# thu-pacman/chitu

Hardware: AMD Instinct MI355X
Metric: output tok/s (bs=16) DeepSeek-R1 FP8 TP=8; HBM GB/s vs peak (higher is better)
Workload: dtype fp8_e4m3 weights+activations (W8A8, fp32 accumulate), bf16 attention

## Files before the change

chitu_amd/csrc/moe.hip:

```cpp
#include "common.h"
#include "gemm_common.h"
#ifndef CHITU_MOE_PROBE_MASK
#define CHITU_MOE_PROBE_MASK 0
#endif

namespace chitu {

struct MoeStage {
    W8Frag w;
    i32x4 x[2];
    float xs, ws;
};

__device__ __forceinline__ void moe_store_tile(bf16_t* out_row, int n0, int g, int N, const f32x4& acc, float rw) {
#pragma unroll
    for (int h = 0; h < 2; ++h) {
        const int n = n0 + h * 8 + 2 * g;
        const uint16_t a = f32_to_bf16(acc[2 * h] * rw), b = f32_to_bf16(acc[2 * h + 1] * rw);
        if (n + 1 < N && (N & 1) == 0) *reinterpret_cast<uint32_t*>(out_row + n) = (uint32_t)a | ((uint32_t)b << 16);
        else {
            if (n < N) out_row[n] = a;
            if (n + 1 < N) out_row[n + 1] = b;
        }
    }
}

__device__ __forceinline__ float moe_routed_weight(const void* topk_w, int w_dt, int slot) {
    if (w_dt == 0) return bf16_to_f32(((const bf16_t*)topk_w)[slot]);
    if (w_dt == 1) return f16_to_f32(((const uint16_t*)topk_w)[slot]);
    return ((const float*)topk_w)[slot];
}

template <int WK, int NW, int D>
__global__ __launch_bounds__(64 * WK * NW) void moe_gemm1_kernel(
    const fp8_t* __restrict__ Xq, const float* __restrict__ Xs, const fp8_t* __restrict__ W,
    const float* __restrict__ Ws, const int32_t* __restrict__ sorted_ids,
    const int32_t* __restrict__ expert_ids, const int32_t* __restrict__ num_post_pad,
    bf16_t* __restrict__ out, int numel, int topk, int N, int K) {
    static_assert(WK == 1 || NW == 1, "either split K or tile N inside a workgroup");
    __shared__ float red[WK > 1 ? WK * 256 : 1];
    const int mb = blockIdx.y;
    if (mb * 16 >= *num_post_pad) return;
    const int lane = threadIdx.x & 63, wave = __builtin_amdgcn_readfirstlane(threadIdx.x >> 6);
    const int j = lane & 15, g = lane >> 4;
    const int n0 = (NW > 1 ? blockIdx.x * NW + wave : blockIdx.x) * 16;
    if (NW > 1 && n0 >= N) return;
    const int KB = K >> 7;
    const int slot = sorted_ids[mb * 16 + j];
    const bool valid = slot < numel;
    const int e = expert_ids[mb];
    f32x4 acc = f32x4{0.f, 0.f, 0.f, 0.f};
    if (e >= 0) {
        const int kw = NW > 1 ? 0 : wave;
        const int kb0 = KB * kw / WK, kb1 = KB * (kw + 1) / WK;
        const int slot0 = __builtin_amdgcn_readfirstlane(slot);
        const int token = (valid ? slot : min(slot0, numel - 1)) / topk;
        const fp8_t* xp = Xq + (size_t)token * K + g * 16;
        const float* xsp = Xs + (size_t)token * KB;
        const fp8_t *wp0, *wp1;
        w8_lane_ptrs(W + (size_t)e * N * K, n0, N, K, j, g, wp0, wp1);
        const float* wsp = Ws + ((size_t)e * ((N + 127) >> 7) + (n0 >> 7)) * KB;
        auto load = [&](MoeStage& st, int kb) {
            const int off = kb << 7;
            st.w.w[0] = __builtin_nontemporal_load(reinterpret_cast<const i32x4*>(wp0 + off));
            st.w.w[1] = __builtin_nontemporal_load(reinterpret_cast<const i32x4*>(wp1 + off));
            st.x[0] = *reinterpret_cast<const i32x4*>(xp + off);
            st.x[1] = *reinterpret_cast<const i32x4*>(xp + off + 64);
            st.xs = xsp[kb];
            st.ws = wsp[kb];
        };
        auto compute = [&](const MoeStage& st) {
            const f32x4 blk = w8a8_block_dot(st.w, st.x[0], st.x[1]);
#pragma unroll
            for (int r = 0; r < 4; ++r) acc[r] += (blk[r] * st.xs) * st.ws;
        };
        MoeStage ring[D];
#pragma unroll
        for (int d = 0; d < D; ++d)
            if (kb0 + d < kb1) load(ring[d], kb0 + d);
        for (int kb = kb0; kb < kb1; kb += D) {
#pragma unroll
            for (int d = 0; d < D; ++d) {
                if (kb + d < kb1) {
                    compute(ring[d]);
                    if (kb + d + D < kb1) load(ring[d], kb + d + D);
                }
            }
        }
    }
    if (WK > 1) {
        *reinterpret_cast<f32x4*>(&red[(wave * 64 + lane) * 4]) = acc;
        __syncthreads();
        if (wave != 0) return;
        acc = f32x4{0.f, 0.f, 0.f, 0.f};
#pragma unroll
        for (int w = 0; w < WK; ++w) {
            const f32x4 v = *reinterpret_cast<const f32x4*>(&red[(w * 64 + lane) * 4]);
#pragma unroll
            for (int r = 0; r < 4; ++r) acc[r] += v[r];
        }
    }
    if (!valid) return;
    moe_store_tile(out + (size_t)slot * N, n0, g, N, acc, 1.0f);
}

struct MoeStage2 {
    W8Frag wg, wu;
    i32x4 x[2];
    float xs, wsg, wsu;
};

template <int WK, int D, bool Q = false>
__global__ __launch_bounds__(Q ? 512 : 64 * WK) void moe_gemm1_silu_kernel(
    const fp8_t* __restrict__ Xq, const float* __restrict__ Xs, const fp8_t* __restrict__ W,
    const float* __restrict__ Ws, const int32_t* __restrict__ sorted_ids,
    const int32_t* __restrict__ expert_ids, const int32_t* __restrict__ num_post_pad,
    bf16_t* __restrict__ out, int numel, int topk, int I, int K, fp8_t* __restrict__ hq = nullptr,
    float* __restrict__ hs = nullptr, float eps = 0.f) {
    static_assert(!Q || WK == 1, "the quantising epilogue owns whole K");
    __shared__ float red[WK > 1 ? WK * 512 : 1];
    __shared__ float qmax[Q ? 8 * 16 : 1];
    const int mb = blockIdx.y;
    if (mb * 16 >= *num_post_pad) return;
    const int lane = threadIdx.x & 63;
    const int wave_id = __builtin_amdgcn_readfirstlane(threadIdx.x >> 6);
    const int wave = Q ? 0 : wave_id;
    const int j = lane & 15, g = lane >> 4;
    const int n0 = (Q ? blockIdx.x * 8 + wave_id : blockIdx.x) * 16;
    const int N = 2 * I;
    const int KB = K >> 7;
    const int slot = sorted_ids[mb * 16 + j];
    const bool valid = slot < numel;
    const int e = expert_ids[mb];
    f32x4 ag = f32x4{0.f, 0.f, 0.f, 0.f}, au = f32x4{0.f, 0.f, 0.f, 0.f};
    if (e >= 0) {
        const int kb0 = KB * wave / WK, kb1 = KB * (wave + 1) / WK;
        const int slot0 = __builtin_amdgcn_readfirstlane(slot);
        const int token = (valid ? slot : min(slot0, numel - 1)) / topk;
        const fp8_t* xp = Xq + (size_t)token * K + g * 16;
        const float* xsp = Xs + (size_t)token * KB;
        if (CHITU_MOE_PROBE_MASK & 1) {
            xp = Xq + (size_t)(g * 16 + (token & 15)) * 16;
            xsp = Xs + (token & 15);
        }
        const fp8_t* Wb = W + (size_t)e * N * K;
        const fp8_t *gp0, *gp1, *up0, *up1;
        w8_lane_ptrs(Wb, n0, N, K, j, g, gp0, gp1);
        w8_lane_ptrs(Wb, I + n0, N, K, j, g, up0, up1);
        const float* wsb = Ws + (size_t)e * ((N + 127) >> 7) * KB;
        const float* wsgp = wsb + (size_t)(n0 >> 7) * KB;
        const float* wsup = wsb + (size_t)((I + n0) >> 7) * KB;
        auto load = [&](MoeStage2& st, int kb) {
            const int off = kb << 7;
            st.wg.w[0] = __builtin_nontemporal_load(reinterpret_cast<const i32x4*>(gp0 + off));
            st.wg.w[1] = __builtin_nontemporal_load(reinterpret_cast<const i32x4*>(gp1 + off));
            st.wu.w[0] = __builtin_nontemporal_load(reinterpret_cast<const i32x4*>(up0 + off));
            st.wu.w[1] = __builtin_nontemporal_load(reinterpret_cast<const i32x4*>(up1 + off));
            if (CHITU_MOE_PROBE_MASK & 1) {
                st.x[0] = *reinterpret_cast<const i32x4*>(xp + (size_t)kb * 2048);
                st.x[1] = *reinterpret_cast<const i32x4*>(xp + (size_t)kb * 2048 + 1024);
                st.xs = xsp[kb * 16];
            } else {
                st.x[0] = *reinterpret_cast<const i32x4*>(xp + off);
                st.x[1] = *reinterpret_cast<const i32x4*>(xp + off + 64);
                st.xs = xsp[kb];
            }
            st.wsg = wsgp[kb];
            st.wsu = wsup[kb];
        };
        auto compute = [&](const MoeStage2& st) {
            const f32x4 bg = w8a8_block_dot(st.wg, st.x[0], st.x[1]);
            const f32x4 bu = w8a8_block_dot(st.wu, st.x[0], st.x[1]);
#pragma unroll
            for (int r = 0; r < 4; ++r) {
                ag[r] += (bg[r] * st.xs) * st.wsg;
                au[r] += (bu[r] * st.xs) * st.wsu;
            }
        };
        MoeStage2 ring[D];
#pragma unroll
        for (int d = 0; d < D; ++d)
            if (kb0 + d < kb1) load(ring[d], kb0 + d);
        for (int kb = kb0; kb < kb1; kb += D) {
#pragma unroll
            for (int d = 0; d < D; ++d) {
                if (kb + d < kb1) {
                    compute(ring[d]);
                    if (kb + d + D < kb1) load(ring[d], kb + d + D);
                }
            }
        }
    }
    if (WK > 1) {
        *reinterpret_cast<f32x4*>(&red[(wave * 128 + lane) * 4]) = ag;
        *reinterpret_cast<f32x4*>(&red[(wave * 128 + 64 + lane) * 4]) = au;
        __syncthreads();
        if (wave != 0) return;
        ag = f32x4{0.f, 0.f, 0.f, 0.f};
        au = f32x4{0.f, 0.f, 0.f, 0.f};
#pragma unroll
        for (int w = 0; w < WK; ++w) {
            const f32x4 vg = *reinterpret_cast<const f32x4*>(&red[(w * 128 + lane) * 4]);
            const f32x4 vu = *reinterpret_cast<const f32x4*>(&red[(w * 128 + 64 + lane) * 4]);
#pragma unroll
            for (int r = 0; r < 4; ++r) {
                ag[r] += vg[r];
                au[r] += vu[r];
            }
        }
    }
    if (!Q && !valid) return;
    f32x4 h;
#pragma unroll
    for (int r = 0; r < 4; ++r) {
        const float gv = round_bf16(ag[r]), uv = round_bf16(au[r]);
        const float sl = round_bf16(gv / (1.0f + expf(-gv)));
        h[r] = round_bf16(sl * uv);
    }
    if (!Q) {
        moe_store_tile(out + (size_t)slot * I, n0, g, I, h, 1.0f);
        return;
    }
    float amax = __builtin_fmaxf(__builtin_fmaxf(__builtin_fabsf(h[0]), __builtin_fabsf(h[1])),
                                 __builtin_fmaxf(__builtin_fabsf(h[2]), __builtin_fabsf(h[3])));
    amax = __builtin_fmaxf(amax, __shfl_xor(amax, 16, 64));
    amax = __builtin_fmaxf(amax, __shfl_xor(amax, 32, 64));
    if (g == 0) qmax[wave_id * 16 + j] = amax;
    __syncthreads();
    amax = qmax[j];
#pragma unroll
    for (int w = 1; w < 8; ++w) amax = __builtin_fmaxf(amax, qmax[w * 16 + j]);
    const float sc = __builtin_fmaxf(amax, eps) / 448.0f;
    const float v[8] = {h[0], h[1], h[2], h[3], 0.f, 0.f, 0.f, 0.f};
    const uint32_t codes = (uint32_t)quant8_fp8<true>(v, sc)[0];
    if (!valid) return;
    fp8_t* qrow = hq + (size_t)slot * I + n0 + 2 * g;
    *reinterpret_cast<uint16_t*>(qrow) = (uint16_t)(codes & 0xffffu);
    *reinterpret_cast<uint16_t*>(qrow + 8) = (uint16_t)(codes >> 16);
    if (wave_id == 0 && g == 0) hs[(size_t)slot * (I >> 7) + blockIdx.x] = sc;
}

__global__ __launch_bounds__(256) void moe_silu_quant_kernel(const bf16_t* __restrict__ c1,
                                                             fp8_t* __restrict__ q,
                                                             float* __restrict__ s, int64_t rows,
                                                             int I, float eps, int act_rule) {
    const int lane16 = threadIdx.x & 15;
    const int gpr = I >> 7;
    const int64_t n_groups = rows * gpr;
    int64_t group = ((int64_t)blockIdx.x * blockDim.x + threadIdx.x) >> 4;
    const int64_t stride = ((int64_t)gridDim.x * blockDim.x) >> 4;
    for (; group < n_groups; group += stride) {
        const int64_t row = group / gpr;
        const int col = (int)(group % gpr) * 128 + lane16 * 8;
        const i32x4 graw = *reinterpret_cast<const i32x4*>(c1 + row * 2 * I + col);
        const i32x4 uraw = *reinterpret_cast<const i32x4*>(c1 + row * 2 * I + I + col);
        float h[8];
        float amax = 0.f;
#pragma unroll
        for (int i = 0; i < 8; ++i) {
            const uint32_t gu = (uint32_t)graw[i >> 1], uu = (uint32_t)uraw[i >> 1];
            const float gv = (i & 1) ? __uint_as_float(gu & 0xffff0000u) : __uint_as_float(gu << 16);
            const float uv = (i & 1) ? __uint_as_float(uu & 0xffff0000u) : __uint_as_float(uu << 16);
            const float sl = round_bf16(gv / (1.0f + expf(-gv)));
            h[i] = round_bf16(sl * uv);
            amax = __builtin_fmaxf(amax, __builtin_fabsf(h[i]));
        }
        amax = row16_reduce_max(amax);
        if (!act_rule) amax = __builtin_fmaxf(amax, eps);
        const float sc = amax / 448.0f;
        const i32x2 o = act_rule ? quant8_fp8<false>(h, sc) : quant8_fp8<true>(h, sc);
        *reinterpret_cast<i32x2*>(q + row * I + col) = o;
        if (lane16 == 0) s[group] = sc;
    }
}

template <int KBMAX, int NT>
__global__ __launch_bounds__(256) void moe_gemm2_kernel(
    const fp8_t* __restrict__ Hq, const float* __restrict__ Hs, const fp8_t* __restrict__ W,
    const float* __restrict__ Ws, const int32_t* __restrict__ sorted_ids,
    const int32_t* __restrict__ expert_ids, const int32_t* __restrict__ num_post_pad,
    const void* __restrict__ topk_w, int w_dt, bf16_t* __restrict__ out, int numel, int N, int I,
    int mul_weight) {
    const int mb = blockIdx.y;
    if (mb * 16 >= *num_post_pad) return;
    const int lane = threadIdx.x & 63, wave = __builtin_amdgcn_readfirstlane(threadIdx.x >> 6);
    const int j = lane & 15, g = lane >> 4;
    const int KB = I >> 7;
    const int slot = sorted_ids[mb * 16 + j];
    const bool valid = slot < numel;
    const int e = expert_ids[mb];
    const int row = valid ? slot : 0;
    const float rw = (mul_weight && valid) ? moe_routed_weight(topk_w, w_dt, slot) : 1.0f;
    i32x4 x[KBMAX][2];
    float xs[KBMAX];
    if (e >= 0) {
        const fp8_t* xp = Hq + (size_t)row * I + g * 16;
#pragma unroll
        for (int kb = 0; kb < KBMAX; ++kb) {
            if (kb < KB) {
                x[kb][0] = *reinterpret_cast<const i32x4*>(xp + (kb << 7));
                x[kb][1] = *reinterpret_cast<const i32x4*>(xp + (kb << 7) + 64);
                xs[kb] = Hs[(size_t)row * KB + kb];
            }
        }
    }
    const int tile0 = (blockIdx.x * 4 + wave) * NT;
    W8Frag wf[NT][KBMAX];
    if (e >= 0) {
#pragma unroll
        for (int t = 0; t < NT; ++t) {
            const int n0 = (tile0 + t) * 16;
            if (n0 < N) {
                const fp8_t *wp0, *wp1;
                w8_lane_ptrs(W + (size_t)e * N * I, n0, N, I, j, g, wp0, wp1);
#pragma unroll
                for (int kb = 0; kb < KBMAX; ++kb) {
                    if (kb < KB) {
                        wf[t][kb].w[0] = __builtin_nontemporal_load(reinterpret_cast<const i32x4*>(wp0 + (kb << 7)));
                        wf[t][kb].w[1] = __builtin_nontemporal_load(reinterpret_cast<const i32x4*>(wp1 + (kb << 7)));
                    }
                }
            }
        }
    }
#pragma unroll
    for (int t = 0; t < NT; ++t) {
        const int n0 = (tile0 + t) * 16;
        if (n0 >= N) break;
        f32x4 acc = f32x4{0.f, 0.f, 0.f, 0.f};
        if (e >= 0) {
            const float* wsp = Ws + ((size_t)e * ((N + 127) >> 7) + (n0 >> 7)) * KB;
#pragma unroll
            for (int kb = 0; kb < KBMAX; ++kb) {
                if (kb < KB) {
                    const f32x4 blk = w8a8_block_dot(wf[t][kb], x[kb][0], x[kb][1]);
                    const float ws = wsp[kb];
#pragma unroll
                    for (int r = 0; r < 4; ++r) acc[r] += (blk[r] * xs[kb]) * ws;
                }
            }
        }
        if (valid) moe_store_tile(out + (size_t)slot * N, n0, g, N, acc, rw);
    }
}

template <int KB, int NT, int ROUNDS>
__global__ __launch_bounds__(256) void moe_gemm2_q_kernel(
    const bf16_t* __restrict__ Hb, const fp8_t* __restrict__ W, const float* __restrict__ Ws,
    const int32_t* __restrict__ sorted_ids, const int32_t* __restrict__ expert_ids,
    const int32_t* __restrict__ num_post_pad, const void* __restrict__ topk_w, int w_dt,
    bf16_t* __restrict__ out, int numel, int N, int mul_weight, float eps) {
    constexpr int I = KB * 128;
    constexpr int HPW = (2 * KB + 3) / 4;
    __shared__ float amax_lds[2 * KB][16];
    __shared__ i32x4 xq_lds[2 * KB][64];
    const int mb = blockIdx.y;
    if (mb * 16 >= *num_post_pad) return;
    const int lane = threadIdx.x & 63, wave = __builtin_amdgcn_readfirstlane(threadIdx.x >> 6);
    const int j = lane & 15, g = lane >> 4;
    const int slot = sorted_ids[mb * 16 + j];
    const bool valid = slot < numel;
    const int e = expert_ids[mb];
    auto tile_of = [&](int r) { return ((blockIdx.x * ROUNDS + r) * 4 + wave) * NT; };
    if (e < 0) {
#pragma unroll
        for (int r = 0; r < ROUNDS; ++r)
#pragma unroll
            for (int t = 0; t < NT; ++t) {
                const int n0 = (tile_of(r) + t) * 16;
                if (n0 < N && valid) moe_store_tile(out + (size_t)slot * N, n0, g, N, f32x4{0.f, 0.f, 0.f, 0.f}, 1.0f);
            }
        return;
    }
    const int row = valid ? slot : 0;
    const bf16_t* hrow = Hb + (size_t)row * I;
    i32x4 hraw[HPW][2];
#pragma unroll
    for (int q = 0; q < HPW; ++q) {
        const int hb = min(wave + 4 * q, 2 * KB - 1);
        hraw[q][0] = *reinterpret_cast<const i32x4*>(hrow + hb * 64 + g * 16);
        hraw[q][1] = *reinterpret_cast<const i32x4*>(hrow + hb * 64 + g * 16 + 8);
    }
    const int last_tile = (N - 1) >> 4;
    const fp8_t* We = W + (size_t)e * N * I;
    W8Frag wf[ROUNDS > 1 ? 2 : 1][NT][KB];
    auto load_round = [&](W8Frag (&dst)[NT][KB], int r) {
#pragma unroll
        for (int t = 0; t < NT; ++t) {
            const int n0 = min(tile_of(r) + t, last_tile) * 16;
            const fp8_t *wp0, *wp1;
            w8_lane_ptrs(We, n0, N, I, j, g, wp0, wp1);
#pragma unroll
            for (int kb = 0; kb < KB; ++kb) {
                dst[t][kb].w[0] = __builtin_nontemporal_load(reinterpret_cast<const i32x4*>(wp0 + (kb << 7)));
                dst[t][kb].w[1] = __builtin_nontemporal_load(reinterpret_cast<const i32x4*>(wp1 + (kb << 7)));
            }
        }
    };
    load_round(wf[0], 0);
    const float rw = (mul_weight && valid) ? moe_routed_weight(topk_w, w_dt, slot) : 1.0f;
    float h[HPW][16];
#pragma unroll
    for (int q = 0; q < HPW; ++q) {
        const int hb = wave + 4 * q;
        float amax = 0.f;
#pragma unroll
        for (int i = 0; i < 16; ++i) {
            const uint32_t u = (uint32_t)hraw[q][i >> 3][(i >> 1) & 3];
            h[q][i] = (i & 1) ? __uint_as_float(u & 0xffff0000u) : __uint_as_float(u << 16);
            amax = __builtin_fmaxf(amax, __builtin_fabsf(h[q][i]));
        }
        amax = __builtin_fmaxf(amax, __shfl_xor(amax, 16, 64));
        amax = __builtin_fmaxf(amax, __shfl_xor(amax, 32, 64));
        if (g == 0 && hb < 2 * KB) amax_lds[hb][j] = amax;
    }
    __syncthreads();
#pragma unroll
    for (int q = 0; q < HPW; ++q) {
        const int hb = wave + 4 * q;
        if (hb < 2 * KB) {
            const float sc = __builtin_fmaxf(__builtin_fmaxf(amax_lds[hb & ~1][j], amax_lds[hb | 1][j]), eps) / 448.0f;
            float lo[8], hi[8];
#pragma unroll
            for (int i = 0; i < 8; ++i) {
                lo[i] = h[q][i];
                hi[i] = h[q][8 + i];
            }
            const i32x2 a = quant8_fp8<true>(lo, sc), b = quant8_fp8<true>(hi, sc);
            xq_lds[hb][lane] = i32x4{a[0], a[1], b[0], b[1]};
        }
    }
    __syncthreads();
    i32x4 x[KB][2];
    float xs[KB];
#pragma unroll
    for (int kb = 0; kb < KB; ++kb) {
        x[kb][0] = xq_lds[2 * kb][lane];
        x[kb][1] = xq_lds[2 * kb + 1][lane];
        xs[kb] = __builtin_fmaxf(__builtin_fmaxf(amax_lds[2 * kb][j], amax_lds[2 * kb + 1][j]), eps) / 448.0f;
    }
    const float* wse = Ws + (size_t)e * ((N + 127) >> 7) * KB;
#pragma unroll
    for (int r = 0; r < ROUNDS; ++r) {
        if (r + 1 < ROUNDS) load_round(wf[(r + 1) & 1], r + 1);
#pragma unroll
        for (int t = 0; t < NT; ++t) {
            const int n0 = (tile_of(r) + t) * 16;
            f32x4 acc = f32x4{0.f, 0.f, 0.f, 0.f};
            const float* wsp = wse + (size_t)(min(n0, N - 1) >> 7) * KB;
#pragma unroll
            for (int kb = 0; kb < KB; ++kb) {
                const f32x4 blk = w8a8_block_dot(wf[r & 1][t][kb], x[kb][0], x[kb][1]);
                const float ws = wsp[kb];
#pragma unroll
                for (int rr = 0; rr < 4; ++rr) acc[rr] += (blk[rr] * xs[kb]) * ws;
            }
            if (valid && n0 < N) moe_store_tile(out + (size_t)slot * N, n0, g, N, acc, rw);
        }
    }
}

template <int WK>
__global__ __launch_bounds__(64 * WK) void moe_gemm2_generic_kernel(
    const fp8_t* __restrict__ Hq, const float* __restrict__ Hs, const fp8_t* __restrict__ W,
    const float* __restrict__ Ws, const int32_t* __restrict__ sorted_ids,
    const int32_t* __restrict__ expert_ids, const int32_t* __restrict__ num_post_pad,
    const void* __restrict__ topk_w, int w_dt, bf16_t* __restrict__ out, int numel, int N, int I,
    int mul_weight) {
    __shared__ float red[WK > 1 ? WK * 256 : 1];
    const int mb = blockIdx.y;
    if (mb * 16 >= *num_post_pad) return;
    const int lane = threadIdx.x & 63, wave = __builtin_amdgcn_readfirstlane(threadIdx.x >> 6);
    const int j = lane & 15, g = lane >> 4;
    const int n0 = blockIdx.x * 16;
    const int KB = I >> 7;
    const int slot = sorted_ids[mb * 16 + j];
    const bool valid = slot < numel;
    const int e = expert_ids[mb];
    const int row = valid ? slot : 0;
    f32x4 acc = f32x4{0.f, 0.f, 0.f, 0.f};
    if (e >= 0) {
        const int kb0 = KB * wave / WK, kb1 = KB * (wave + 1) / WK;
        const fp8_t* xp = Hq + (size_t)row * I + g * 16;
        const float* xsp = Hs + (size_t)row * KB;
        const fp8_t *wp0, *wp1;
        w8_lane_ptrs(W + (size_t)e * N * I, n0, N, I, j, g, wp0, wp1);
        const float* wsp = Ws + ((size_t)e * ((N + 127) >> 7) + (n0 >> 7)) * KB;
        for (int kb = kb0; kb < kb1; ++kb) {
            const int off = kb << 7;
            W8Frag f;
            f.w[0] = __builtin_nontemporal_load(reinterpret_cast<const i32x4*>(wp0 + off));
            f.w[1] = __builtin_nontemporal_load(reinterpret_cast<const i32x4*>(wp1 + off));
            const i32x4 x0 = *reinterpret_cast<const i32x4*>(xp + off);
            const i32x4 x1 = *reinterpret_cast<const i32x4*>(xp + off + 64);
            const f32x4 blk = w8a8_block_dot(f, x0, x1);
            const float xs = xsp[kb], ws = wsp[kb];
#pragma unroll
            for (int r = 0; r < 4; ++r) acc[r] += (blk[r] * xs) * ws;
        }
    }
    if (WK > 1) {
        *reinterpret_cast<f32x4*>(&red[(wave * 64 + lane) * 4]) = acc;
        __syncthreads();
        if (wave != 0) return;
        acc = f32x4{0.f, 0.f, 0.f, 0.f};
#pragma unroll
        for (int w = 0; w < WK; ++w) {
            const f32x4 v = *reinterpret_cast<const f32x4*>(&red[(w * 64 + lane) * 4]);
#pragma unroll
            for (int r = 0; r < 4; ++r) acc[r] += v[r];
        }
    }
    if (!valid) return;
    const float rw = mul_weight ? moe_routed_weight(topk_w, w_dt, slot) : 1.0f;
    moe_store_tile(out + (size_t)slot * N, n0, g, N, acc, rw);
}

__global__ __launch_bounds__(256) void moe_sum_kernel(const bf16_t* __restrict__ c3,
                                                      bf16_t* __restrict__ out, int64_t M, int topk,
                                                      int64_t N) {
    const int64_t n8 = N >> 3;
    for (int64_t idx = (int64_t)blockIdx.x * blockDim.x + threadIdx.x; idx < M * n8;
         idx += (int64_t)gridDim.x * blockDim.x) {
        const int64_t t = idx / n8, c = (idx % n8) * 8;
        float acc[8] = {0.f, 0.f, 0.f, 0.f, 0.f, 0.f, 0.f, 0.f};
        for (int k = 0; k < topk; ++k) {
            const i32x4 raw = *reinterpret_cast<const i32x4*>(c3 + (t * topk + k) * N + c);
#pragma unroll
            for (int i = 0; i < 4; ++i) {
                const uint32_t u = (uint32_t)raw[i];
                acc[2 * i] += __uint_as_float(u << 16);
                acc[2 * i + 1] += __uint_as_float(u & 0xffff0000u);
            }
        }
        i32x4 o;
#pragma unroll
        for (int i = 0; i < 4; ++i)
            o[i] = (int)((uint32_t)f32_to_bf16(acc[2 * i]) | ((uint32_t)f32_to_bf16(acc[2 * i + 1]) << 16));
        *reinterpret_cast<i32x4*>(out + t * N + c) = o;
    }
}

}

extern "C" int chitu_hip_moe_gemm1_fp8(const void* a_fp8, const float* a_scale, const void* w1_fp8,
                                       const float* w1_scale, const int32_t* sorted_token_ids,
                                       const int32_t* expert_ids,
                                       const int32_t* num_tokens_post_pad, void* out_bf16,
                                       int64_t numel, int32_t topk, int64_t N, int64_t K,
                                       int64_t max_mblocks, void* stream) {
    using namespace chitu;
    CHITU_REQUIRE(a_fp8 && a_scale && w1_fp8 && w1_scale && sorted_token_ids && expert_ids);
    CHITU_REQUIRE(num_tokens_post_pad && out_bf16);
    CHITU_REQUIRE(numel >= 0 && topk >= 1 && N >= 1 && K >= 128 && max_mblocks >= 0);
    if (K % 128 != 0) return CHITU_ERR_UNSUPPORTED;
    if (numel == 0 || max_mblocks == 0) return CHITU_OK;
    const int n_tiles = (int)((N + 15) / 16);
    const dim3 grid((unsigned)n_tiles, (unsigned)max_mblocks);
    const int64_t wgs = (int64_t)n_tiles * (numel < max_mblocks ? numel : max_mblocks);
    const int KB = (int)(K / 128);
    int WK = wgs <= 512 ? 8 : wgs <= 1024 ? 4 : wgs <= 2048 ? 2 : 1;
// ... 188 lines not shown
```

chitu_amd/csrc/moe_bf16.hip:

```cpp
#include "common.h"
#include "gemm_common.h"

namespace chitu {

constexpr int kWBf16 = 0, kWSoftFp8 = 1;

template <int WKIND>
struct MoeBfStage {
    i32x4 w[2];
    s16x8 x[WKIND == kWSoftFp8 ? 4 : 2];
    float ws;
};

template <int WKIND>
struct MoeBfAcc {
    f32x4 e0, o0, e1, o1;
    __device__ __forceinline__ void zero() { e0 = o0 = e1 = o1 = f32x4{0.f, 0.f, 0.f, 0.f}; }
    __device__ __forceinline__ f32x4 fold() const { return f32x4{e0[0] + o0[1], e0[2] + o0[3], e1[0] + o1[1], e1[2] + o1[3]}; }
};

template <int WKIND>
__device__ __forceinline__ void moe_bf_mma(MoeBfAcc<WKIND>& a, const i32x4 (&w)[2], const s16x8* x, float ws) {
    if (WKIND == kWBf16) {
        const s16x8 w0 = __builtin_bit_cast(s16x8, w[0]), w1 = __builtin_bit_cast(s16x8, w[1]);
        a.e0 = __builtin_amdgcn_mfma_f32_16x16x32_bf16(w0, x[0], a.e0, 0, 0, 0);
        a.o0 = __builtin_amdgcn_mfma_f32_16x16x32_bf16(w0, x[1], a.o0, 0, 0, 0);
        a.e1 = __builtin_amdgcn_mfma_f32_16x16x32_bf16(w1, x[0], a.e1, 0, 0, 0);
        a.o1 = __builtin_amdgcn_mfma_f32_16x16x32_bf16(w1, x[1], a.o1, 0, 0, 0);
    } else {
        const float s2 = ws * __uint_as_float(0x7B800000u);
#pragma unroll
        for (int h = 0; h < 2; ++h) {
            const s16x8 wa = soft_decode8((uint32_t)w[h][0], (uint32_t)w[h][1], s2);
            const s16x8 wb = soft_decode8((uint32_t)w[h][2], (uint32_t)w[h][3], s2);
            f32x4& e = h == 0 ? a.e0 : a.e1;
            f32x4& o = h == 0 ? a.o0 : a.o1;
            e = __builtin_amdgcn_mfma_f32_16x16x32_bf16(wa, x[0], e, 0, 0, 0);
            e = __builtin_amdgcn_mfma_f32_16x16x32_bf16(wb, x[1], e, 0, 0, 0);
            o = __builtin_amdgcn_mfma_f32_16x16x32_bf16(wa, x[2], o, 0, 0, 0);
            o = __builtin_amdgcn_mfma_f32_16x16x32_bf16(wb, x[3], o, 0, 0, 0);
        }
    }
}

template <int WKIND, int WK, bool SILU>
__global__ __launch_bounds__(64 * WK) void moe_gemm_bf16_kernel(
    const bf16_t* __restrict__ X, const void* __restrict__ Wv, const float* __restrict__ Ws,
    const int32_t* __restrict__ sorted_ids, const int32_t* __restrict__ expert_ids,
    const int32_t* __restrict__ num_post_pad, const void* __restrict__ topk_w, int w_dt, int mul_routed,
    bf16_t* __restrict__ out, int numel, int a_div, int N_out, int K) {
    constexpr int kTiles = SILU ? 2 : 1;
    __shared__ float red[WK > 1 ? WK * kTiles * 256 : 1];
    const int mb = blockIdx.y;
    if (mb * 16 >= *num_post_pad) return;
    const int lane = threadIdx.x & 63, wave = __builtin_amdgcn_readfirstlane(threadIdx.x >> 6);
    const int j = lane & 15, g = lane >> 4;
    const int n0 = blockIdx.x * 16;
    const int Nw = SILU ? 2 * N_out : N_out;
    constexpr int kBlk = WKIND == kWSoftFp8 ? 128 : 64;
    constexpr int kEl = WKIND == kWSoftFp8 ? 1 : 2;
    const int KB = K / kBlk;
    const int slot = sorted_ids[mb * 16 + j];
    const bool valid = slot < numel;
    const int e = expert_ids[mb];
    MoeBfAcc<WKIND> acc[kTiles];
#pragma unroll
    for (int t = 0; t < kTiles; ++t) acc[t].zero();
    if (e >= 0) {
        const int kb0 = KB * wave / WK, kb1 = KB * (wave + 1) / WK;
        const int slot0 = __builtin_amdgcn_readfirstlane(slot);
        const int row = (valid ? slot : min(slot0, numel - 1)) / a_div;
        const bf16_t* xp = X + (size_t)row * K + g * (WKIND == kWSoftFp8 ? 16 : 8);
        const uint8_t* Wb = (const uint8_t*)Wv + (size_t)e * Nw * K * kEl;
        const int loff = ((j & 1) * 4 + g) * 16;
        const uint8_t* wp[kTiles][2];
        const float* wsp[kTiles];
#pragma unroll
        for (int t = 0; t < kTiles; ++t) {
            const int base = t * N_out + n0, lim = t * N_out + N_out - 1;
            wp[t][0] = Wb + (size_t)min(base + (j >> 1), lim) * K * kEl + loff;
            wp[t][1] = Wb + (size_t)min(base + 8 + (j >> 1), lim) * K * kEl + loff;
            wsp[t] = WKIND == kWSoftFp8 ? Ws + ((size_t)e * ((Nw + 127) >> 7) + (base >> 7)) * KB : nullptr;
        }
        constexpr int D = SILU ? 2 : 3;
        MoeBfStage<WKIND> ring[D][kTiles];
        auto load = [&](MoeBfStage<WKIND> (&st)[kTiles], int kb) {
            const size_t off = (size_t)kb * 128;
#pragma unroll
            for (int t = 0; t < kTiles; ++t) {
                st[t].w[0] = __builtin_nontemporal_load(reinterpret_cast<const i32x4*>(wp[t][0] + off));
                st[t].w[1] = __builtin_nontemporal_load(reinterpret_cast<const i32x4*>(wp[t][1] + off));
                st[t].ws = WKIND == kWSoftFp8 ? wsp[t][kb] : 1.0f;
            }
            const bf16_t* xk = xp + (size_t)kb * kBlk;
            if (WKIND == kWSoftFp8) {
                st[0].x[0] = *reinterpret_cast<const s16x8*>(xk);
                st[0].x[1] = *reinterpret_cast<const s16x8*>(xk + 8);
                st[0].x[2] = *reinterpret_cast<const s16x8*>(xk + 64);
                st[0].x[3] = *reinterpret_cast<const s16x8*>(xk + 72);
            } else {
                st[0].x[0] = *reinterpret_cast<const s16x8*>(xk);
                st[0].x[1] = *reinterpret_cast<const s16x8*>(xk + 32);
            }
        };
        auto compute = [&](const MoeBfStage<WKIND> (&st)[kTiles]) {
#pragma unroll
            for (int t = 0; t < kTiles; ++t) moe_bf_mma<WKIND>(acc[t], st[t].w, st[0].x, st[t].ws);
        };
#pragma unroll
        for (int d = 0; d < D; ++d)
            if (kb0 + d < kb1) load(ring[d], kb0 + d);
        for (int kb = kb0; kb < kb1; kb += D) {
#pragma unroll
            for (int d = 0; d < D; ++d) {
                if (kb + d < kb1) {
                    compute(ring[d]);
                    if (kb + d + D < kb1) load(ring[d], kb + d + D);
                }
            }
        }
    }
    f32x4 r[kTiles];
#pragma unroll
    for (int t = 0; t < kTiles; ++t) r[t] = acc[t].fold();
    if (WK > 1) {
#pragma unroll
        for (int t = 0; t < kTiles; ++t) *reinterpret_cast<f32x4*>(&red[((wave * kTiles + t) * 64 + lane) * 4]) = r[t];
        __syncthreads();
        if (wave != 0) return;
#pragma unroll
        for (int t = 0; t < kTiles; ++t) {
            r[t] = f32x4{0.f, 0.f, 0.f, 0.f};
#pragma unroll
            for (int w = 0; w < WK; ++w) {
                const f32x4 v = *reinterpret_cast<const f32x4*>(&red[((w * kTiles + t) * 64 + lane) * 4]);
#pragma unroll
                for (int i = 0; i < 4; ++i) r[t][i] += v[i];
            }
        }
    }
    if (!valid) return;
    f32x4 res = r[0];
    float rw = 1.0f;
    if (SILU) {
#pragma unroll
        for (int i = 0; i < 4; ++i) {
            const float gv = round_bf16(r[0][i]), uv = round_bf16(r[1][i]);
// ... 67 lines not shown
```

chitu_amd/csrc/moe_int8.hip:

```cpp
#include "common.h"
#include "gemm_common.h"

namespace chitu {

typedef int i32x4m __attribute__((ext_vector_type(4)));

struct I8Stage2 {
    i32x4m wg[2], wu[2], x[2];
};
struct I8Stage1 {
    i32x4m w[2], x[2];
};

__device__ __forceinline__ i32x4m i8_combine(const i32x4m& e0, const i32x4m& o0, const i32x4m& e1, const i32x4m& o1) {
    return i32x4m{e0[0] + o0[1], e0[2] + o0[3], e1[0] + o1[1], e1[2] + o1[3]};
}

__device__ __forceinline__ void i8_store_tile(bf16_t* row, int n0, int g, int N, const float (&v)[4]) {
#pragma unroll
    for (int h = 0; h < 2; ++h) {
        const int n = n0 + h * 8 + 2 * g;
        if (n + 1 < N && (N & 1) == 0) *reinterpret_cast<uint32_t*>(row + n) = f32x2_to_bf16x2(v[2 * h], v[2 * h + 1]);
        else {
            if (n < N) row[n] = f32_to_bf16(v[2 * h]);
            if (n + 1 < N) row[n + 1] = f32_to_bf16(v[2 * h + 1]);
        }
    }
}

template <int WK>
__global__ __launch_bounds__(64 * WK) void moe_i8_gemm1_silu_kernel(
    const int8_t* __restrict__ Xq, const float* __restrict__ Xs, const int8_t* __restrict__ W,
    const float* __restrict__ Ws, const int32_t* __restrict__ sorted_ids, const int32_t* __restrict__ expert_ids,
    const int32_t* __restrict__ num_post_pad, bf16_t* __restrict__ out, int numel, int topk, int I, int K) {
    __shared__ int red[WK > 1 ? WK * 512 : 1];
    const int mb = blockIdx.y;
    if (mb * 16 >= *num_post_pad) return;
    const int lane = threadIdx.x & 63, wave = __builtin_amdgcn_readfirstlane(threadIdx.x >> 6);
    const int j = lane & 15, g = lane >> 4;
    const int n0 = blockIdx.x * 16;
    const int N = 2 * I;
    const int KB = K >> 7;
    const int slot = sorted_ids[mb * 16 + j];
    const bool valid = slot < numel;
    const int e = expert_ids[mb];
    const int slot0 = __builtin_amdgcn_readfirstlane(slot);
    const int token = (valid ? slot : min(slot0, numel - 1)) / topk;
    i32x4m ge0 = {0, 0, 0, 0}, go0 = ge0, ge1 = ge0, go1 = ge0, ue0 = ge0, uo0 = ge0, ue1 = ge0, uo1 = ge0;
    if (e >= 0) {
        const int kb0 = KB * wave / WK, kb1 = KB * (wave + 1) / WK;
        const int8_t* xp = Xq + (size_t)token * K + g * 16;
        const fp8_t* Wb = reinterpret_cast<const fp8_t*>(W) + (size_t)e * N * K;
        const fp8_t *gp0, *gp1, *up0, *up1;
        w8_lane_ptrs(Wb, n0, N, K, j, g, gp0, gp1);
        w8_lane_ptrs(Wb, I + n0, N, K, j, g, up0, up1);
        auto load = [&](I8Stage2& st, int kb) {
            const int off = kb << 7;
            st.wg[0] = __builtin_nontemporal_load(reinterpret_cast<const i32x4m*>(gp0 + off));
            st.wg[1] = __builtin_nontemporal_load(reinterpret_cast<const i32x4m*>(gp1 + off));
            st.wu[0] = __builtin_nontemporal_load(reinterpret_cast<const i32x4m*>(up0 + off));
            st.wu[1] = __builtin_nontemporal_load(reinterpret_cast<const i32x4m*>(up1 + off));
            st.x[0] = *reinterpret_cast<const i32x4m*>(xp + off);
            st.x[1] = *reinterpret_cast<const i32x4m*>(xp + off + 64);
        };
        auto compute = [&](const I8Stage2& st) {
            ge0 = __builtin_amdgcn_mfma_i32_16x16x64_i8(st.wg[0], st.x[0], ge0, 0, 0, 0);
            go0 = __builtin_amdgcn_mfma_i32_16x16x64_i8(st.wg[0], st.x[1], go0, 0, 0, 0);
            ge1 = __builtin_amdgcn_mfma_i32_16x16x64_i8(st.wg[1], st.x[0], ge1, 0, 0, 0);
            go1 = __builtin_amdgcn_mfma_i32_16x16x64_i8(st.wg[1], st.x[1], go1, 0, 0, 0);
            ue0 = __builtin_amdgcn_mfma_i32_16x16x64_i8(st.wu[0], st.x[0], ue0, 0, 0, 0);
            uo0 = __builtin_amdgcn_mfma_i32_16x16x64_i8(st.wu[0], st.x[1], uo0, 0, 0, 0);
            ue1 = __builtin_amdgcn_mfma_i32_16x16x64_i8(st.wu[1], st.x[0], ue1, 0, 0, 0);
            uo1 = __builtin_amdgcn_mfma_i32_16x16x64_i8(st.wu[1], st.x[1], uo1, 0, 0, 0);
        };
        constexpr int D = 3;
        I8Stage2 ring[D];
#pragma unroll
        for (int d = 0; d < D; ++d)
            if (kb0 + d < kb1) load(ring[d], kb0 + d);
        for (int kb = kb0; kb < kb1; kb += D) {
#pragma unroll
            for (int d = 0; d < D; ++d) {
                if (kb + d < kb1) {
                    compute(ring[d]);
                    if (kb + d + D < kb1) load(ring[d], kb + d + D);
                }
            }
        }
    }
    i32x4m ag = i8_combine(ge0, go0, ge1, go1), au = i8_combine(ue0, uo0, ue1, uo1);
    if (WK > 1) {
        *reinterpret_cast<i32x4m*>(&red[(wave * 128 + lane) * 4]) = ag;
        *reinterpret_cast<i32x4m*>(&red[(wave * 128 + 64 + lane) * 4]) = au;
        __syncthreads();
        if (wave != 0) return;
        ag = au = i32x4m{0, 0, 0, 0};
#pragma unroll
        for (int w = 0; w < WK; ++w) {
            const i32x4m vg = *reinterpret_cast<const i32x4m*>(&red[(w * 128 + lane) * 4]);
            const i32x4m vu = *reinterpret_cast<const i32x4m*>(&red[(w * 128 + 64 + lane) * 4]);
#pragma unroll
            for (int r = 0; r < 4; ++r) {
                ag[r] += vg[r];
                au[r] += vu[r];
            }
        }
    }
    if (!valid) return;
    const float sx = Xs[token];
    const float* wse = Ws + (size_t)max(e, 0) * N;
    float h[4];
#pragma unroll
    for (int r = 0; r < 4; ++r) {
        const int n = w8_out_col(n0, g, r);
        const int nc = min(n, I - 1);
        const float gv = e >= 0 ? round_bf16(((float)ag[r] * sx) * wse[nc]) : 0.f;
        const float uv = e >= 0 ? round_bf16(((float)au[r] * sx) * wse[I + nc]) : 0.f;
        h[r] = round_bf16(gv / (1.0f + expf(-gv))) * uv;
    }
    i8_store_tile(out + (size_t)slot * I, n0, g, I, h);
}

template <int WK>
__global__ __launch_bounds__(64 * WK) void moe_i8_gemm2_kernel(
    const int8_t* __restrict__ Aq, const float* __restrict__ As, const int8_t* __restrict__ W,
    const float* __restrict__ Ws, const int32_t* __restrict__ sorted_ids, const int32_t* __restrict__ expert_ids,
    const int32_t* __restrict__ num_post_pad, const void* __restrict__ topk_w, int w_dt, bf16_t* __restrict__ out,
    int numel, int N, int I, int mul_weight) {
    __shared__ int red[WK > 1 ? WK * 256 : 1];
    const int mb = blockIdx.y;
    if (mb * 16 >= *num_post_pad) return;
    const int lane = threadIdx.x & 63, wave = __builtin_amdgcn_readfirstlane(threadIdx.x >> 6);
    const int j = lane & 15, g = lane >> 4;
    const int n0 = blockIdx.x * 16;
    const int KB = I >> 7;
    const int slot = sorted_ids[mb * 16 + j];
    const bool valid = slot < numel;
    const int e = expert_ids[mb];
    const int row = valid ? slot : 0;
    i32x4m e0 = {0, 0, 0, 0}, o0 = e0, e1 = e0, o1 = e0;
    if (e >= 0) {
        const int kb0 = KB * wave / WK, kb1 = KB * (wave + 1) / WK;
        const int8_t* xp = Aq + (size_t)row * I + g * 16;
        const fp8_t *wp0, *wp1;
        w8_lane_ptrs(reinterpret_cast<const fp8_t*>(W) + (size_t)e * N * I, n0, N, I, j, g, wp0, wp1);
        auto load = [&](I8Stage1& st, int kb) {
            const int off = kb << 7;
            st.w[0] = __builtin_nontemporal_load(reinterpret_cast<const i32x4m*>(wp0 + off));
            st.w[1] = __builtin_nontemporal_load(reinterpret_cast<const i32x4m*>(wp1 + off));
            st.x[0] = *reinterpret_cast<const i32x4m*>(xp + off);
            st.x[1] = *reinterpret_cast<const i32x4m*>(xp + off + 64);
        };
        auto compute = [&](const I8Stage1& st) {
            e0 = __builtin_amdgcn_mfma_i32_16x16x64_i8(st.w[0], st.x[0], e0, 0, 0, 0);
            o0 = __builtin_amdgcn_mfma_i32_16x16x64_i8(st.w[0], st.x[1], o0, 0, 0, 0);
            e1 = __builtin_amdgcn_mfma_i32_16x16x64_i8(st.w[1], st.x[0], e1, 0, 0, 0);
            o1 = __builtin_amdgcn_mfma_i32_16x16x64_i8(st.w[1], st.x[1], o1, 0, 0, 0);
        };
        constexpr int D = 4;
        I8Stage1 ring[D];
#pragma unroll
        for (int d = 0; d < D; ++d)
            if (kb0 + d < kb1) load(ring[d], kb0 + d);
        for (int kb = kb0; kb < kb1; kb += D) {
#pragma unroll
            for (int d = 0; d < D; ++d) {
                if (kb + d < kb1) {
                    compute(ring[d]);
                    if (kb + d + D < kb1) load(ring[d], kb + d + D);
                }
            }
        }
    }
    i32x4m acc = i8_combine(e0, o0, e1, o1);
    if (WK > 1) {
        *reinterpret_cast<i32x4m*>(&red[(wave * 64 + lane) * 4]) = acc;
        __syncthreads();
        if (wave != 0) return;
        acc = i32x4m{0, 0, 0, 0};
#pragma unroll
        for (int w = 0; w < WK; ++w) {
            const i32x4m v = *reinterpret_cast<const i32x4m*>(&red[(w * 64 + lane) * 4]);
#pragma unroll
            for (int r = 0; r < 4; ++r) acc[r] += v[r];
        }
    }
    if (!valid) return;
    float rw = 1.0f;
    if (mul_weight)
        rw = w_dt == 0 ? bf16_to_f32(((const bf16_t*)topk_w)[slot]) : w_dt == 1 ? f16_to_f32(((const uint16_t*)topk_w)[slot]) : ((const float*)topk_w)[slot];
    const float sa = As[row];
    const float* wse = Ws + (size_t)max(e, 0) * N;
    float y[4];
#pragma unroll
    for (int r = 0; r < 4; ++r) {
        const int n = min(w8_out_col(n0, g, r), N - 1);
        y[r] = e >= 0 ? round_bf16(((float)acc[r] * sa) * wse[n]) * rw : 0.f;
    }
    i8_store_tile(out + (size_t)slot * N, n0, g, N, y);
}

static int pick_wk(int64_t wgs, int KB) {
    int WK = wgs <= 640 ? 8 : 4;
    if (KB < 16) WK = wgs <= 640 ? 8 : wgs <= 1536 ? 4 : wgs <= 3200 ? 2 : 1;
    debug_override(kOptMoeI8WK, WK);
    while (WK > 1 && WK > KB) WK >>= 1;
    return WK;
}

}

extern "C" int chitu_hip_moe_i8_gemm1_silu(const void* a_int8, const float* a_scale, const void* w1_int8,
                                           const float* w1_scale, const int32_t* sorted_token_ids,
                                           const int32_t* expert_ids, const int32_t* num_tokens_post_pad,
                                           void* h_bf16, int64_t numel, int32_t topk, int64_t inter_size, int64_t K,
                                           int64_t max_mblocks, void* stream) {
    using namespace chitu;
    CHITU_REQUIRE(a_int8 && a_scale && w1_int8 && w1_scale && sorted_token_ids && expert_ids && num_tokens_post_pad && h_bf16);
    CHITU_REQUIRE(numel >= 0 && topk >= 1 && inter_size >= 16 && K >= 128 && max_mblocks >= 0);
    if (K % 128 != 0 || inter_size % 16 != 0) return CHITU_ERR_UNSUPPORTED;
    if (numel == 0 || max_mblocks == 0) return CHITU_OK;
// ... 39 lines not shown
```

Before: 205.7.

## Hoist MoE block-head loads and issue expert weight prefetch before token gathers

Adds a shared block-head helper that loads num_post_pad and expert_ids together into scalar registers, and fetches the 16 sorted slot ids with one vector load instead of per-lane gathers. In the fused gate/up SiLU kernel and the quantising down-projection kernel, expert weight loads are issued before the dependent token-index and activation loads, so HBM weight streaming starts without waiting on the slot-to-token chain. The down-projection kernel also gets a deeper weight prefetch ring plus an occupancy hint in launch_bounds. The costs are higher register pressure, which may lower occupancy or cause spills, and inline-asm ties that constrain the compiler's scheduling.

```diff
diff --git a/chitu_amd/csrc/moe.hip b/chitu_amd/csrc/moe.hip
--- a/chitu_amd/csrc/moe.hip
+++ b/chitu_amd/csrc/moe.hip
@@ -1,5 +1,6 @@
 #include "common.h"
 #include "gemm_common.h"
+#include "moe_head.h"
 #ifndef CHITU_MOE_PROBE_MASK
 #define CHITU_MOE_PROBE_MASK 0
 #endif
@@ -40,15 +41,15 @@
     static_assert(WK == 1 || NW == 1, "either split K or tile N inside a workgroup");
     __shared__ float red[WK > 1 ? WK * 256 : 1];
     const int mb = blockIdx.y;
-    if (mb * 16 >= *num_post_pad) return;
+    int e;
+    if (!moe_block_head(expert_ids, num_post_pad, mb, e)) return;
     const int lane = threadIdx.x & 63, wave = __builtin_amdgcn_readfirstlane(threadIdx.x >> 6);
     const int j = lane & 15, g = lane >> 4;
     const int n0 = (NW > 1 ? blockIdx.x * NW + wave : blockIdx.x) * 16;
     if (NW > 1 && n0 >= N) return;
     const int KB = K >> 7;
-    const int slot = sorted_ids[mb * 16 + j];
+    const int slot = moe_block_slot(sorted_ids, mb, j);
     const bool valid = slot < numel;
-    const int e = expert_ids[mb];
     f32x4 acc = f32x4{0.f, 0.f, 0.f, 0.f};
     if (e >= 0) {
         const int kw = NW > 1 ? 0 : wave;
@@ -121,7 +122,9 @@
     __shared__ float red[WK > 1 ? WK * 512 : 1];
     __shared__ float qmax[Q ? 8 * 16 : 1];
     const int mb = blockIdx.y;
-    if (mb * 16 >= *num_post_pad) return;
+    int e;
+    if (!moe_block_head(expert_ids, num_post_pad, mb, e, Xq, Xs, W, Ws, sorted_ids, numel, topk, I, K)) return;
+    const i32x16u ids = moe_block_slots(sorted_ids, mb);
     const int lane = threadIdx.x & 63;
     const int wave_id = __builtin_amdgcn_readfirstlane(threadIdx.x >> 6);
     const int wave = Q ? 0 : wave_id;
@@ -129,45 +132,54 @@
     const int n0 = (Q ? blockIdx.x * 8 + wave_id : blockIdx.x) * 16;
     const int N = 2 * I;
     const int KB = K >> 7;
-    const int slot = sorted_ids[mb * 16 + j];
+    f32x4 ag = f32x4{0.f, 0.f, 0.f, 0.f}, au = f32x4{0.f, 0.f, 0.f, 0.f};
+    const int kb0 = KB * wave / WK, kb1 = KB * (wave + 1) / WK;
+    const fp8_t *gp0, *gp1, *up0, *up1, *xp;
+    const float *wsgp, *wsup, *xsp;
+    auto load_w = [&](MoeStage2& st, int kb) {
+        const int off = kb << 7;
+        st.wg.w[0] = __builtin_nontemporal_load(reinterpret_cast<const i32x4*>(gp0 + off));
+        st.wg.w[1] = __builtin_nontemporal_load(reinterpret_cast<const i32x4*>(gp1 + off));
+        st.wu.w[0] = __builtin_nontemporal_load(reinterpret_cast<const i32x4*>(up0 + off));
+        st.wu.w[1] = __builtin_nontemporal_load(reinterpret_cast<const i32x4*>(up1 + off));
+        st.wsg = wsgp[kb];
+        st.wsu = wsup[kb];
+    };
+    auto load_x = [&](MoeStage2& st, int kb) {
+        const int off = kb << 7;
+        if (CHITU_MOE_PROBE_MASK & 1) {
+            st.x[0] = *reinterpret_cast<const i32x4*>(xp + (size_t)kb * 2048);
+            st.x[1] = *reinterpret_cast<const i32x4*>(xp + (size_t)kb * 2048 + 1024);
+            st.xs = xsp[kb * 16];
+        } else {
+            st.x[0] = *reinterpret_cast<const i32x4*>(xp + off);
+            st.x[1] = *reinterpret_cast<const i32x4*>(xp + off + 64);
+            st.xs = xsp[kb];
+        }
+    };
+    MoeStage2 ring[D];
+    if (e >= 0) {
+        const fp8_t* Wb = W + (size_t)e * N * K;
+        w8_lane_ptrs(Wb, n0, N, K, j, g, gp0, gp1);
+        w8_lane_ptrs(Wb, I + n0, N, K, j, g, up0, up1);
+        const float* wsb = Ws + (size_t)e * ((N + 127) >> 7) * KB;
+        wsgp = wsb + (size_t)(n0 >> 7) * KB;
+        wsup = wsb + (size_t)((I + n0) >> 7) * KB;
+#pragma unroll
+        for (int d = 0; d < D; ++d)
+            if (kb0 + d < kb1) load_w(ring[d], kb0 + d);
+    }
+    const int slot = moe_slot_of_lane(ids, j);
     const bool valid = slot < numel;
-    const int e = expert_ids[mb];
-    f32x4 ag = f32x4{0.f, 0.f, 0.f, 0.f}, au = f32x4{0.f, 0.f, 0.f, 0.f};
     if (e >= 0) {
-        const int kb0 = KB * wave / WK, kb1 = KB * (wave + 1) / WK;
         const int slot0 = __builtin_amdgcn_readfirstlane(slot);
         const int token = (valid ? slot : min(slot0, numel - 1)) / topk;
-        const fp8_t* xp = Xq + (size_t)token * K + g * 16;
-        const float* xsp = Xs + (size_t)token * KB;
+        xp = Xq + (size_t)token * K + g * 16;
+        xsp = Xs + (size_t)token * KB;
         if (CHITU_MOE_PROBE_MASK & 1) {
             xp = Xq + (size_t)(g * 16 + (token & 15)) * 16;
             xsp = Xs + (token & 15);
         }
-        const fp8_t* Wb = W + (size_t)e * N * K;
-        const fp8_t *gp0, *gp1, *up0, *up1;
-        w8_lane_ptrs(Wb, n0, N, K, j, g, gp0, gp1);
-        w8_lane_ptrs(Wb, I + n0, N, K, j, g, up0, up1);
-        const float* wsb = Ws + (size_t)e * ((N + 127) >> 7) * KB;
-        const float* wsgp = wsb + (size_t)(n0 >> 7) * KB;
-        const float* wsup = wsb + (size_t)((I + n0) >> 7) * KB;
-        auto load = [&](MoeStage2& st, int kb) {
-            const int off = kb << 7;
-            st.wg.w[0] = __builtin_nontemporal_load(reinterpret_cast<const i32x4*>(gp0 + off));
-            st.wg.w[1] = __builtin_nontemporal_load(reinterpret_cast<const i32x4*>(gp1 + off));
-            st.wu.w[0] = __builtin_nontemporal_load(reinterpret_cast<const i32x4*>(up0 + off));
-            st.wu.w[1] = __builtin_nontemporal_load(reinterpret_cast<const i32x4*>(up1 + off));
-            if (CHITU_MOE_PROBE_MASK & 1) {
-                st.x[0] = *reinterpret_cast<const i32x4*>(xp + (size_t)kb * 2048);
-                st.x[1] = *reinterpret_cast<const i32x4*>(xp + (size_t)kb * 2048 + 1024);
-                st.xs = xsp[kb * 16];
-            } else {
-                st.x[0] = *reinterpret_cast<const i32x4*>(xp + off);
-                st.x[1] = *reinterpret_cast<const i32x4*>(xp + off + 64);
-                st.xs = xsp[kb];
-            }
-            st.wsg = wsgp[kb];
-            st.wsu = wsup[kb];
-        };
         auto compute = [&](const MoeStage2& st) {
             const f32x4 bg = w8a8_block_dot(st.wg, st.x[0], st.x[1]);
             const f32x4 bu = w8a8_block_dot(st.wu, st.x[0], st.x[1]);
@@ -177,16 +189,18 @@
                 au[r] += (bu[r] * st.xs) * st.wsu;
             }
         };
-        MoeStage2 ring[D];
 #pragma unroll
         for (int d = 0; d < D; ++d)
-            if (kb0 + d < kb1) load(ring[d], kb0 + d);
+            if (kb0 + d < kb1) load_x(ring[d], kb0 + d);
         for (int kb = kb0; kb < kb1; kb += D) {
 #pragma unroll
             for (int d = 0; d < D; ++d) {
                 if (kb + d < kb1) {
                     compute(ring[d]);
-                    if (kb + d + D < kb1) load(ring[d], kb + d + D);
+                    if (kb + d + D < kb1) {
+                        load_w(ring[d], kb + d + D);
+                        load_x(ring[d], kb + d + D);
+                    }
                 }
             }
         }
@@ -282,13 +296,13 @@
     const void* __restrict__ topk_w, int w_dt, bf16_t* __restrict__ out, int numel, int N, int I,
     int mul_weight) {
     const int mb = blockIdx.y;
-    if (mb * 16 >= *num_post_pad) return;
+    int e;
+    if (!moe_block_head(expert_ids, num_post_pad, mb, e)) return;
     const int lane = threadIdx.x & 63, wave = __builtin_amdgcn_readfirstlane(threadIdx.x >> 6);
     const int j = lane & 15, g = lane >> 4;
     const int KB = I >> 7;
-    const int slot = sorted_ids[mb * 16 + j];
+    const int slot = moe_block_slot(sorted_ids, mb, j);
     const bool valid = slot < numel;
-    const int e = expert_ids[mb];
     const int row = valid ? slot : 0;
     const float rw = (mul_weight && valid) ? moe_routed_weight(topk_w, w_dt, slot) : 1.0f;
     i32x4 x[KBMAX][2];
@@ -345,7 +359,7 @@
 }
 
 template <int KB, int NT, int ROUNDS>
-__global__ __launch_bounds__(256) void moe_gemm2_q_kernel(
+__global__ __launch_bounds__(256, NT <= 2 ? 3 : 1) void moe_gemm2_q_kernel(
     const bf16_t* __restrict__ Hb, const fp8_t* __restrict__ W, const float* __restrict__ Ws,
     const int32_t* __restrict__ sorted_ids, const int32_t* __restrict__ expert_ids,
     const int32_t* __restrict__ num_post_pad, const void* __restrict__ topk_w, int w_dt,
@@ -355,24 +369,51 @@
     __shared__ float amax_lds[2 * KB][16];
     __shared__ i32x4 xq_lds[2 * KB][64];
     const int mb = blockIdx.y;
-    if (mb * 16 >= *num_post_pad) return;
+    int e;
+    if (!moe_block_head(expert_ids, num_post_pad, mb, e, Hb, W, Ws, sorted_ids, topk_w, w_dt, out, numel, N, mul_weight)) return;
+    const i32x16u ids = moe_block_slots(sorted_ids, mb);
     const int lane = threadIdx.x & 63, wave = __builtin_amdgcn_readfirstlane(threadIdx.x >> 6);
     const int j = lane & 15, g = lane >> 4;
-    const int slot = sorted_ids[mb * 16 + j];
-    const bool valid = slot < numel;
-    const int e = expert_ids[mb];
     auto tile_of = [&](int r) { return ((blockIdx.x * ROUNDS + r) * 4 + wave) * NT; };
     if (e < 0) {
+        const int slot = moe_slot_of_lane(ids, j);
 #pragma unroll
         for (int r = 0; r < ROUNDS; ++r)
 #pragma unroll
             for (int t = 0; t < NT; ++t) {
                 const int n0 = (tile_of(r) + t) * 16;
-                if (n0 < N && valid) moe_store_tile(out + (size_t)slot * N, n0, g, N, f32x4{0.f, 0.f, 0.f, 0.f}, 1.0f);
+                if (n0 < N && slot < numel) moe_store_tile(out + (size_t)slot * N, n0, g, N, f32x4{0.f, 0.f, 0.f, 0.f}, 1.0f);
             }
         return;
     }
+    const int last_tile = (N - 1) >> 4;
+    const fp8_t* We = W + (size_t)e * N * I;
+    constexpr int PF = NT <= 2 ? (ROUNDS > 2 ? 2 : ROUNDS - 1) : (ROUNDS > 1 ? 1 : 0);
+    constexpr int WFD = PF + 1;
+    W8Frag wf[WFD][NT][KB];
+    auto load_round = [&](W8Frag (&dst)[NT][KB], int r) {
+#pragma unroll
+        for (int t = 0; t < NT; ++t) {
+            const int n0 = min(tile_of(r) + t, last_tile) * 16;
+            const fp8_t *wp0, *wp1;
+            w8_lane_ptrs(We, n0, N, I, j, g, wp0, wp1);
+#pragma unroll
+            for (int kb = 0; kb < KB; ++kb) {
+                dst[t][kb].w[0] = __builtin_nontemporal_load(reinterpret_cast<const i32x4*>(wp0 + (kb << 7)));
+                dst[t][kb].w[1] = __builtin_nontemporal_load(reinterpret_cast<const i32x4*>(wp1 + (kb << 7)));
+            }
+        }
+    };
+    load_round(wf[0], 0);
+    if (PF >= 2) load_round(wf[1], 1);
+    const int slot = moe_slot_of_lane(ids, j);
+    const bool valid = slot < numel;
     const int row = valid ? slot : 0;
+    uint32_t rw_bits;
+    if (mul_weight) {
+        if (w_dt == 2) rw_bits = ((const uint32_t*)topk_w)[row];
+        else rw_bits = ((const uint16_t*)topk_w)[row];
+    }
     const bf16_t* hrow = Hb + (size_t)row * I;
     i32x4 hraw[HPW][2];
 #pragma unroll
@@ -381,24 +422,6 @@
         hraw[q][0] = *reinterpret_cast<const i32x4*>(hrow + hb * 64 + g * 16);
         hraw[q][1] = *reinterpret_cast<const i32x4*>(hrow + hb * 64 + g * 16 + 8);
     }
-    const int last_tile = (N - 1) >> 4;
-    const fp8_t* We = W + (size_t)e * N * I;
-    W8Frag wf[ROUNDS > 1 ? 2 : 1][NT][KB];
-    auto load_round = [&](W8Frag (&dst)[NT][KB], int r) {
-#pragma unroll
-        for (int t = 0; t < NT; ++t) {
-            const int n0 = min(tile_of(r) + t, last_tile) * 16;
-            const fp8_t *wp0, *wp1;
-            w8_lane_ptrs(We, n0, N, I, j, g, wp0, wp1);
-#pragma unroll
-            for (int kb = 0; kb < KB; ++kb) {
-                dst[t][kb].w[0] = __builtin_nontemporal_load(reinterpret_cast<const i32x4*>(wp0 + (kb << 7)));
-                dst[t][kb].w[1] = __builtin_nontemporal_load(reinterpret_cast<const i32x4*>(wp1 + (kb << 7)));
-            }
-        }
-    };
-    load_round(wf[0], 0);
-    const float rw = (mul_weight && valid) ? moe_routed_weight(topk_w, w_dt, slot) : 1.0f;
     float h[HPW][16];
 #pragma unroll
     for (int q = 0; q < HPW; ++q) {
@@ -440,9 +463,11 @@
         xs[kb] = __builtin_fmaxf(__builtin_fmaxf(amax_lds[2 * kb][j], amax_lds[2 * kb + 1][j]), eps) / 448.0f;
     }
     const float* wse = Ws + (size_t)e * ((N + 127) >> 7) * KB;
+    float rw = 1.0f;
+    if (mul_weight && valid) rw = w_dt == 0 ? __uint_as_float(rw_bits << 16) : w_dt == 1 ? f16_to_f32((uint16_t)rw_bits) : __uint_as_float(rw_bits);
 #pragma unroll
     for (int r = 0; r < ROUNDS; ++r) {
-        if (r + 1 < ROUNDS) load_round(wf[(r + 1) & 1], r + 1);
+        if (PF >= 1 && r + PF < ROUNDS) load_round(wf[(r + PF) % WFD], r + PF);
 #pragma unroll
         for (int t = 0; t < NT; ++t) {
             const int n0 = (tile_of(r) + t) * 16;
@@ -450,7 +475,7 @@
             const float* wsp = wse + (size_t)(min(n0, N - 1) >> 7) * KB;
 #pragma unroll
             for (int kb = 0; kb < KB; ++kb) {
-                const f32x4 blk = w8a8_block_dot(wf[r & 1][t][kb], x[kb][0], x[kb][1]);
+                const f32x4 blk = w8a8_block_dot(wf[r % WFD][t][kb], x[kb][0], x[kb][1]);
                 const float ws = wsp[kb];
 #pragma unroll
                 for (int rr = 0; rr < 4; ++rr) acc[rr] += (blk[rr] * xs[kb]) * ws;
@@ -469,14 +494,14 @@
     int mul_weight) {
     __shared__ float red[WK > 1 ? WK * 256 : 1];
     const int mb = blockIdx.y;
-    if (mb * 16 >= *num_post_pad) return;
+    int e;
+    if (!moe_block_head(expert_ids, num_post_pad, mb, e)) return;
     const int lane = threadIdx.x & 63, wave = __builtin_amdgcn_readfirstlane(threadIdx.x >> 6);
     const int j = lane & 15, g = lane >> 4;
     const int n0 = blockIdx.x * 16;
     const int KB = I >> 7;
-    const int slot = sorted_ids[mb * 16 + j];
+    const int slot = moe_block_slot(sorted_ids, mb, j);
     const bool valid = slot < numel;
-    const int e = expert_ids[mb];
     const int row = valid ? slot : 0;
     f32x4 acc = f32x4{0.f, 0.f, 0.f, 0.f};
     if (e >= 0) {
diff --git a/chitu_amd/csrc/moe_bf16.hip b/chitu_amd/csrc/moe_bf16.hip
--- a/chitu_amd/csrc/moe_bf16.hip
+++ b/chitu_amd/csrc/moe_bf16.hip
@@ -1,5 +1,6 @@
 #include "common.h"
 #include "gemm_common.h"
+#include "moe_head.h"
 
 namespace chitu {
 
@@ -52,7 +53,8 @@
     constexpr int kTiles = SILU ? 2 : 1;
     __shared__ float red[WK > 1 ? WK * kTiles * 256 : 1];
     const int mb = blockIdx.y;
-    if (mb * 16 >= *num_post_pad) return;
+    int e;
+    if (!moe_block_head(expert_ids, num_post_pad, mb, e)) return;
     const int lane = threadIdx.x & 63, wave = __builtin_amdgcn_readfirstlane(threadIdx.x >> 6);
     const int j = lane & 15, g = lane >> 4;
     const int n0 = blockIdx.x * 16;
@@ -60,9 +62,8 @@
     constexpr int kBlk = WKIND == kWSoftFp8 ? 128 : 64;
     constexpr int kEl = WKIND == kWSoftFp8 ? 1 : 2;
     const int KB = K / kBlk;
-    const int slot = sorted_ids[mb * 16 + j];
+    const int slot = moe_block_slot(sorted_ids, mb, j);
     const bool valid = slot < numel;
-    const int e = expert_ids[mb];
     MoeBfAcc<WKIND> acc[kTiles];
 #pragma unroll
     for (int t = 0; t < kTiles; ++t) acc[t].zero();
diff --git a/chitu_amd/csrc/moe_head.h b/chitu_amd/csrc/moe_head.h
--- /dev/null
+++ b/chitu_amd/csrc/moe_head.h
@@ -0,0 +1,38 @@
+#pragma once
+#include "common.h"
+
+namespace chitu {
+
+template <typename T>
+__device__ __forceinline__ void moe_tie_arg(int& token, const T& v) {
+    asm("" : "+s"(token) : "s"(v));
+}
+template <typename... T>
+__device__ __forceinline__ bool moe_block_head(const int32_t* __restrict__ expert_ids,
+                                               const int32_t* __restrict__ num_post_pad, int mb, int& e,
+                                               const T&... args) {
+    int npp = *num_post_pad;
+    e = expert_ids[mb];
+    asm("" : "+s"(npp), "+s"(e));
+    (moe_tie_arg(npp, args), ...);
+    return mb * 16 < npp;
+}
+
+typedef int i32x16u __attribute__((ext_vector_type(16), aligned(4)));
+
+__device__ __forceinline__ i32x16u moe_block_slots(const int32_t* __restrict__ sorted_ids, int mb) {
+    return *reinterpret_cast<const i32x16u*>(sorted_ids + (size_t)mb * 16);
+}
+
+__device__ __forceinline__ int moe_slot_of_lane(const i32x16u& ids, int j) {
+    int slot = ids[0];
+#pragma unroll
+    for (int i = 1; i < 16; ++i) slot = j == i ? ids[i] : slot;
+    return slot;
+}
+
+__device__ __forceinline__ int moe_block_slot(const int32_t* __restrict__ sorted_ids, int mb, int j) {
+    return moe_slot_of_lane(moe_block_slots(sorted_ids, mb), j);
+}
+
+}
diff --git a/chitu_amd/csrc/moe_int8.hip b/chitu_amd/csrc/moe_int8.hip
--- a/chitu_amd/csrc/moe_int8.hip
+++ b/chitu_amd/csrc/moe_int8.hip
@@ -1,5 +1,6 @@
 #include "common.h"
 #include "gemm_common.h"
+#include "moe_head.h"
 
 namespace chitu {
 
@@ -35,15 +36,15 @@
     const int32_t* __restrict__ num_post_pad, bf16_t* __restrict__ out, int numel, int topk, int I, int K) {
     __shared__ int red[WK > 1 ? WK * 512 : 1];
     const int mb = blockIdx.y;
-    if (mb * 16 >= *num_post_pad) return;
+    int e;
+    if (!moe_block_head(expert_ids, num_post_pad, mb, e)) return;
     const int lane = threadIdx.x & 63, wave = __builtin_amdgcn_readfirstlane(threadIdx.x >> 6);
     const int j = lane & 15, g = lane >> 4;
     const int n0 = blockIdx.x * 16;
     const int N = 2 * I;
     const int KB = K >> 7;
-    const int slot = sorted_ids[mb * 16 + j];
+    const int slot = moe_block_slot(sorted_ids, mb, j);
     const bool valid = slot < numel;
-    const int e = expert_ids[mb];
     const int slot0 = __builtin_amdgcn_readfirstlane(slot);
     const int token = (valid ? slot : min(slot0, numel - 1)) / topk;
     i32x4m ge0 = {0, 0, 0, 0}, go0 = ge0, ge1 = ge0, go1 = ge0, ue0 = ge0, uo0 = ge0, ue1 = ge0, uo1 = ge0;
@@ -129,14 +130,14 @@
     int numel, int N, int I, int mul_weight) {
     __shared__ int red[WK > 1 ? WK * 256 : 1];
     const int mb = blockIdx.y;
-    if (mb * 16 >= *num_post_pad) return;
+    int e;
+    if (!moe_block_head(expert_ids, num_post_pad, mb, e)) return;
     const int lane = threadIdx.x & 63, wave = __builtin_amdgcn_readfirstlane(threadIdx.x >> 6);
     const int j = lane & 15, g = lane >> 4;
     const int n0 = blockIdx.x * 16;
     const int KB = I >> 7;
-    const int slot = sorted_ids[mb * 16 + j];
+    const int slot = moe_block_slot(sorted_ids, mb, j);
     const bool valid = slot < numel;
-    const int e = expert_ids[mb];
     const int row = valid ? slot : 0;
     i32x4m e0 = {0, 0, 0, 0}, o0 = e0, e1 = e0, o1 = e0;
     if (e >= 0) {
```

Result: no change. 205.5 (median of 2 runs) (-0.1%).
